# TimZaman/dotaclient

Hardware: NVIDIA H100
Metric: optimizer_steps_per_sec (higher is better)
Workload: dtype f32

## Files before the change

### dotaclient_b200/csrc/gemm_tf32x3.cu

```cuda
#include "dc_common.cuh"
#include "unit_basic.cuh"

namespace {

constexpr int BM = 128, BN = 128, BK = 32;
constexpr int kStages = 2;
constexpr int kTileBytes = BM * BK * 4;
constexpr int kStageBytes = 4 * kTileBytes;
constexpr int kProducerThreads = 128;
constexpr int kProducerGroups = kStages;
constexpr int kConsumerWarp0 = 4 * kProducerGroups;
constexpr int kConsumerThreads = 256;
constexpr int kThreads = kConsumerWarp0 * 32 + kConsumerThreads;
constexpr int kLdS = BN + 8;
constexpr int kDIn = kUnitFeatures;
constexpr size_t kOffStaging = (size_t)kStages * kStageBytes;
constexpr size_t kOffBars = kOffStaging + (size_t)BM * kLdS * 4;
constexpr size_t kSmemBytes = kOffBars + 128 + 1024 ;

#define DC_ACC8(b) "+f"(d[b]), "+f"(d[b + 1]), "+f"(d[b + 2]), "+f"(d[b + 3]), "+f"(d[b + 4]), "+f"(d[b + 5]), "+f"(d[b + 6]), "+f"(d[b + 7])
__device__ __forceinline__ void wgmma_m64n128k8(float (&d)[64], uint64_t desc_a, uint64_t desc_b) {
    asm volatile(
        "{\n\t.reg .pred p;\n\tsetp.ne.b32 p, %66, 0;\n\t"
        "wgmma.mma_async.sync.aligned.m64n128k8.f32.tf32.tf32 "
        "{%0, %1, %2, %3, %4, %5, %6, %7, %8, %9, %10, %11, %12, %13, %14, %15, "
        "%16, %17, %18, %19, %20, %21, %22, %23, %24, %25, %26, %27, %28, %29, %30, %31, "
        "%32, %33, %34, %35, %36, %37, %38, %39, %40, %41, %42, %43, %44, %45, %46, %47, "
        "%48, %49, %50, %51, %52, %53, %54, %55, %56, %57, %58, %59, %60, %61, %62, %63}, "
        "%64, %65, p, 1, 1;\n\t}\n"
        : DC_ACC8(0), DC_ACC8(8), DC_ACC8(16), DC_ACC8(24), DC_ACC8(32), DC_ACC8(40), DC_ACC8(48), DC_ACC8(56)
        : "l"(desc_a), "l"(desc_b), "r"(1));
}
#undef DC_ACC8

__device__ __forceinline__ void mma_stage(float (&d)[64], uint32_t stage_base, int wg) {
    const uint64_t a_hi = dc_wgmma_desc(stage_base + wg * (64 * 128)), a_lo = dc_wgmma_desc(stage_base + kTileBytes + wg * (64 * 128));
    const uint64_t b_hi = dc_wgmma_desc(stage_base + 2 * kTileBytes), b_lo = dc_wgmma_desc(stage_base + 3 * kTileBytes);
#pragma unroll
    for (int i = 0; i < 64; ++i) dc_reg_fence(d[i]);
    dc_wgmma_fence();
#pragma unroll
    for (int ks = 0; ks < BK / 8; ++ks) {
        const uint64_t adv = (uint64_t)(ks * 2);
        wgmma_m64n128k8(d, a_lo + adv, b_hi + adv);
        wgmma_m64n128k8(d, a_hi + adv, b_lo + adv);
        wgmma_m64n128k8(d, a_hi + adv, b_hi + adv);
    }
    dc_wgmma_commit();
    dc_wgmma_wait0();
#pragma unroll
    for (int i = 0; i < 64; ++i) dc_reg_fence(d[i]);
}

__device__ __forceinline__ void consume(float (&d)[64], unsigned char *tiles, uint64_t *full, uint64_t *empty, uint32_t &c, int n,
                                       int wg, int lane) {
#pragma unroll
    for (int i = 0; i < 64; ++i) d[i] = 0.f;
    for (int kc = 0; kc < n; ++kc, ++c) {
        const int s = c % kStages;
        dc_mbar_wait(&full[s], (c / kStages) & 1);
        __syncwarp();
        mma_stage(d, dc_smem_u32(tiles + (size_t)s * kStageBytes), wg);
        __syncwarp();
        if (lane == 0) dc_mbar_arrive(&empty[s]);
    }
}

__device__ __forceinline__ void consumer_sync() { asm volatile("bar.sync 1, %0;" ::"n"(kConsumerThreads) : "memory"); }

__device__ __forceinline__ void stage_acc(const float (&d)[64], float *S, int ct) {
    const int wg = ct >> 7, w = (ct >> 5) & 3, lane = ct & 31;
    const int r0 = 64 * wg + 16 * w + (lane >> 2), c0 = 2 * (lane & 3);
#pragma unroll
    for (int i = 0; i < 64; i += 2) {
        const int row = r0 + 8 * ((i >> 1) & 1), col = 8 * (i >> 2) + c0;
        *reinterpret_cast<float2 *>(S + row * kLdS + col) = make_float2(d[i], d[i + 1]);
    }
}

__device__ __forceinline__ void init_ring(uint64_t *bars) {
    if (threadIdx.x == 0) {
        for (int s = 0; s < kStages; ++s) { dc_mbar_init(&bars[s], 4); dc_mbar_init(&bars[kStages + s], kConsumerThreads / 32); }
        asm volatile("fence.mbarrier_init.release.cluster;" ::: "memory");
    }
    __syncthreads();
}
__device__ __forceinline__ unsigned char *smem_base(unsigned char *raw) {
    return reinterpret_cast<unsigned char *>((reinterpret_cast<uintptr_t>(raw) + 1023) & ~(uintptr_t)1023);
}
template <typename F>
__device__ __forceinline__ void produce(uint64_t *full, uint64_t *empty, uint32_t c, int lane, F &&store) {
    const int s = c % kStages;
    dc_mbar_wait(&empty[s], ((c / kStages) & 1) ^ 1);
    store(s);
    asm volatile("fence.proxy.async.shared::cta;" ::: "memory");
    __syncwarp();
    if (lane == 0) dc_mbar_arrive(&full[s]);
}

__device__ __forceinline__ void tile_load_k(const float *__restrict__ src, int ld, int row0, int rows_total, int k0, int t,
                                            float4 (&v)[8]) {
    const int c = t & 7, r0 = t >> 3;
#pragma unroll
    for (int i = 0; i < 8; ++i) {
        const int r = r0 + 16 * i;
        v[i] = (row0 + r < rows_total) ? __ldg(reinterpret_cast<const float4 *>(src + (size_t)(row0 + r) * ld + k0) + c)
                                       : make_float4(0.f, 0.f, 0.f, 0.f);
    }
}
__device__ __forceinline__ void tile_store_k(const float4 (&v)[8], unsigned char *dst_hi, unsigned char *dst_lo, int t) {
    const int c = t & 7, r0 = t >> 3;
#pragma unroll
    for (int i = 0; i < 8; ++i) {
        const int r = r0 + 16 * i;
        const int off = r * 128 + ((c ^ (r & 7)) << 4);
        float4 hi, lo;
        hi.x = dc_tf32_rna(v[i].x); hi.y = dc_tf32_rna(v[i].y); hi.z = dc_tf32_rna(v[i].z); hi.w = dc_tf32_rna(v[i].w);
        lo.x = v[i].x - hi.x; lo.y = v[i].y - hi.y; lo.z = v[i].z - hi.z; lo.w = v[i].w - hi.w;
        *reinterpret_cast<float4 *>(dst_hi + off) = hi;
        *reinterpret_cast<float4 *>(dst_lo + off) = lo;
    }
}

template <int NU>
struct DembRaw {
    static constexpr int kP = NU == 16 ? 1 : 2;
    static constexpr int kU = NU == 16 ? 8 : NU;
    float4 d[kP], d2[kP], a[kP];
    uint32_t am[kP];
    float g[kP][kU];
    bool ok[kP];
};
template <>
struct DembRaw<1> {
    float4 v[8];
};

template <int NU>
__device__ __forceinline__ void demb_fetch(DembRaw<NU> &raw, const float *__restrict__ dx, const float *__restrict__ dx2, int ld_dx,
                                           const uint8_t *__restrict__ argmax, const float *__restrict__ dl, int ld_dl,
                                           const float *__restrict__ att, int tok0, int n_tok, int k0, int t) {
    const float4 zero4 = make_float4(0.f, 0.f, 0.f, 0.f);
    if constexpr (NU == 1) {
        const int c = t & 7, r0 = t >> 3;
#pragma unroll
        for (int i = 0; i < 8; ++i) {
            const int n = tok0 + r0 + 16 * i;
            const bool ok = n < n_tok;
            const size_t nn = (size_t)min(n, n_tok - 1);
            float4 d = dx != nullptr ? __ldg(reinterpret_cast<const float4 *>(dx + nn * ld_dx + k0) + c) : zero4;
            if (dx2 != nullptr) {
                const float4 d2 = __ldg(reinterpret_cast<const float4 *>(dx2 + nn * ld_dx + k0) + c);
                d.x += d2.x; d.y += d2.y; d.z += d2.z; d.w += d2.w;
            }
            const float4 a4 = dl != nullptr ? __ldg(reinterpret_cast<const float4 *>(att + nn * 128 + k0) + c) : zero4;
            const float gl = dl != nullptr ? __ldg(dl + nn * ld_dl) : 0.f;
            raw.v[i] = ok ? make_float4(fmaf(gl, a4.x, d.x), fmaf(gl, a4.y, d.y), fmaf(gl, a4.z, d.z), fmaf(gl, a4.w, d.w)) : zero4;
        }
    } else {
        constexpr int kTileToks = (BM - BM % NU) / NU;
#pragma unroll
        for (int k = 0; k < DembRaw<NU>::kP; ++k) {
            const int p = t + kProducerThreads * k;
            const int c = p & 7, tokl = NU == 16 ? p >> 4 : p >> 3;
            const int u0 = NU == 16 ? ((p >> 3) & 1) * 8 : 0;
            const bool active = tokl < kTileToks;
            const int n = tok0 + tokl;
            raw.ok[k] = active && n < n_tok;
            const size_t nn = (size_t)min(n, n_tok - 1);
            float4 d = (active && dx != nullptr) ? __ldg(reinterpret_cast<const float4 *>(dx + nn * ld_dx + k0) + c) : zero4;
            const float4 d2 = (active && dx2 != nullptr) ? __ldg(reinterpret_cast<const float4 *>(dx2 + nn * ld_dx + k0) + c) : zero4;
            if constexpr (NU == 16) {
                raw.d2[k] = d2;
            } else {
                d.x += d2.x; d.y += d2.y; d.z += d2.z; d.w += d2.w;
            }
            raw.d[k] = d;
            raw.am[k] = (active && dx != nullptr) ? __ldg(reinterpret_cast<const uint32_t *>(argmax + nn * 128 + k0) + c) : 0u;
            raw.a[k] = (active && dl != nullptr) ? __ldg(reinterpret_cast<const float4 *>(att + nn * 128 + k0) + c) : zero4;
#pragma unroll
            for (int j = 0; j < DembRaw<NU>::kU; ++j) raw.g[k][j] = (active && dl != nullptr) ? __ldg(dl + nn * ld_dl + u0 + j) : 0.f;
        }
    }
}

__device__ __forceinline__ void store_hi_lo(unsigned char *dst_hi, unsigned char *dst_lo, int off, float4 o) {
    float4 hi, lo;
    hi.x = dc_tf32_rna(o.x); hi.y = dc_tf32_rna(o.y); hi.z = dc_tf32_rna(o.z); hi.w = dc_tf32_rna(o.w);
    lo.x = o.x - hi.x; lo.y = o.y - hi.y; lo.z = o.z - hi.z; lo.w = o.w - hi.w;
    *reinterpret_cast<float4 *>(dst_hi + off) = hi;
    *reinterpret_cast<float4 *>(dst_lo + off) = lo;
}

template <int NU>
__device__ __forceinline__ void demb_store(const DembRaw<NU> &raw, unsigned char *dst_hi, unsigned char *dst_lo, int t) {
    if constexpr (NU == 1) {
        tile_store_k(raw.v, dst_hi, dst_lo, t);
    } else {
        constexpr int kTileRows = BM - BM % NU, kTileToks = kTileRows / NU;
        const float4 zero4 = make_float4(0.f, 0.f, 0.f, 0.f);
#pragma unroll
        for (int k = 0; k < DembRaw<NU>::kP; ++k) {
            const int p = t + kProducerThreads * k;
            const int c = p & 7, tokl = NU == 16 ? p >> 4 : p >> 3;
            const int u0 = NU == 16 ? ((p >> 3) & 1) * 8 : 0;
            if (tokl < kTileToks) {
                float4 d = raw.d[k];
                if constexpr (NU == 16) { d.x += raw.d2[k].x; d.y += raw.d2[k].y; d.z += raw.d2[k].z; d.w += raw.d2[k].w; }
                const float4 a = raw.a[k];
                const uint32_t am = raw.am[k];
#pragma unroll
                for (int j = 0; j < DembRaw<NU>::kU; ++j) {
                    const int u = u0 + j, r = tokl * NU + u;
                    const float gl = raw.g[k][j];
                    float4 o;
                    o.x = fmaf(gl, a.x, (int)(am & 0xffu) == u ? d.x : 0.f);
                    o.y = fmaf(gl, a.y, (int)((am >> 8) & 0xffu) == u ? d.y : 0.f);
                    o.z = fmaf(gl, a.z, (int)((am >> 16) & 0xffu) == u ? d.z : 0.f);
                    o.w = fmaf(gl, a.w, (int)(am >> 24) == u ? d.w : 0.f);
                    store_hi_lo(dst_hi, dst_lo, r * 128 + ((c ^ (r & 7)) << 4), raw.ok[k] ? o : zero4);
                }
            }
        }
        if constexpr (kTileRows < BM) {
            if (t < (BM - kTileRows) * 8) {
                const int r = kTileRows + (t >> 3), c = t & 7;
                store_hi_lo(dst_hi, dst_lo, r * 128 + ((c ^ (r & 7)) << 4), zero4);
            }
        }
    }
}

__device__ __forceinline__ void store_row_k(const float (&v)[32], unsigned char *dst_hi, unsigned char *dst_lo, int row) {
#pragma unroll
    for (int c = 0; c < 8; ++c) {
        const int off = row * 128 + ((c ^ (row & 7)) << 4);
        float4 hi, lo;
        hi.x = dc_tf32_rna(v[4 * c]); hi.y = dc_tf32_rna(v[4 * c + 1]); hi.z = dc_tf32_rna(v[4 * c + 2]); hi.w = dc_tf32_rna(v[4 * c + 3]);
        lo.x = v[4 * c] - hi.x; lo.y = v[4 * c + 1] - hi.y; lo.z = v[4 * c + 2] - hi.z; lo.w = v[4 * c + 3] - hi.w;
        *reinterpret_cast<float4 *>(dst_hi + off) = hi;
        *reinterpret_cast<float4 *>(dst_lo + off) = lo;
    }
}

__global__ void __launch_bounds__(kThreads, 1) gemm_tf32x3_kernel(const float *__restrict__ A, int lda,
                                                                  const float *__restrict__ B, int ldb,
                                                                  const float *__restrict__ bias, float *__restrict__ C,
                                                                  int ldc, int M, int N, int K, int relu, int ksplit,
                                                                  long long c_split_stride) {
    constexpr int kTileRows = BM;
    extern __shared__ unsigned char smem_raw[];
    unsigned char *tiles = smem_base(smem_raw);
    float *S = reinterpret_cast<float *>(tiles + kOffStaging);
    uint64_t *full = reinterpret_cast<uint64_t *>(tiles + kOffBars), *empty = full + kStages;

    const int warp = threadIdx.x >> 5, lane = threadIdx.x & 31;
    const int m_blocks = (M + kTileRows - 1) / kTileRows, n_blocks = (N + BN - 1) / BN, k_chunks = K / BK / ksplit;
    const int tiles_mn = m_blocks * n_blocks, tiles_total = tiles_mn * ksplit;
    init_ring(full);

    if (warp < kConsumerWarp0) {
        const int t = threadIdx.x & (kProducerThreads - 1), g = warp >> 2;
        uint32_t c = 0;
        for (int tile = blockIdx.x; tile < tiles_total; tile += gridDim.x) {
            const int tmn = tile % tiles_mn, kc0 = (tile / tiles_mn) * k_chunks;
            const int m0 = (tmn / n_blocks) * kTileRows, n0 = (tmn % n_blocks) * BN;
            for (int kc = 0; kc < k_chunks; ++kc, ++c) {
                if ((int)(c % kProducerGroups) != g) continue;
                float4 va[8], vb[8];
                tile_load_k(A, lda, m0, M, (kc0 + kc) * BK, t, va);
                tile_load_k(B, ldb, n0, N, (kc0 + kc) * BK, t, vb);
                produce(full, empty, c, lane, [&](int s) {
                    unsigned char *st = tiles + (size_t)s * kStageBytes;
                    tile_store_k(va, st, st + kTileBytes, t);
                    tile_store_k(vb, st + 2 * kTileBytes, st + 3 * kTileBytes, t);
                });
            }
        }
    } else {
        const int ct = threadIdx.x - kConsumerWarp0 * 32, wg = ct >> 7, cw = ct >> 5;
        float d[64];
        uint32_t c = 0;
        for (int tile = blockIdx.x; tile < tiles_total; tile += gridDim.x) {
            const int tmn = tile % tiles_mn, sp = tile / tiles_mn;
            const int m0 = (tmn / n_blocks) * kTileRows, n0 = (tmn % n_blocks) * BN;
            consume(d, tiles, full, empty, c, k_chunks, wg, lane);
            consumer_sync();
            stage_acc(d, S, ct);
            consumer_sync();
            const bool lane_in = n0 + 4 * lane < N;
            const bool has_bias = bias != nullptr && sp == 0 && lane_in;
            const float4 b4 = has_bias ? __ldg(reinterpret_cast<const float4 *>(bias + n0) + lane) : make_float4(0.f, 0.f, 0.f, 0.f);
            float *cbase = C + (size_t)sp * (size_t)c_split_stride + n0 + 4 * lane;
            for (int r = cw; lane_in && r < BM && m0 + r < M; r += kConsumerThreads / 32) {
                float4 v = *reinterpret_cast<const float4 *>(S + r * kLdS + 4 * lane);
                if (has_bias) { v.x += b4.x; v.y += b4.y; v.z += b4.z; v.w += b4.w; }
                if (relu) { v.x = fmaxf(v.x, 0.f); v.y = fmaxf(v.y, 0.f); v.z = fmaxf(v.z, 0.f); v.w = fmaxf(v.w, 0.f); }
                *reinterpret_cast<float4 *>(cbase + (size_t)(m0 + r) * ldc) = v;
            }
        }
    }
}

constexpr int kWsRows = 64;
constexpr int kWsStages = 8;
constexpr int kWsChunkBytes = kWsRows * BK * 4;
constexpr int kWsThreads = kConsumerThreads + 128;
constexpr int kWsLdS = 40;
constexpr size_t kWsOffRing = (size_t)4 * 2 * kTileBytes;
constexpr size_t kWsOffStaging = kWsOffRing + (size_t)kWsStages * kWsChunkBytes;
constexpr size_t kWsOffBars = kWsOffStaging + (size_t)(kConsumerThreads / 32) * 16 * kWsLdS * 4;
constexpr size_t kWsSmemBytes = kWsOffBars + 2 * kWsStages * 8 + 1024 ;
constexpr size_t kWsOffUnits = kWsOffBars + 2 * kWsStages * 8;
constexpr size_t kWsGenSmemBytes = kWsOffUnits + (size_t)4 * kWsRows * kDIn * 4 + 1024 ;
static_assert(kWsSmemBytes <= 227 * 1024 && kWsGenSmemBytes <= 227 * 1024, "weight-stationary GEMM exceeds the shared-memory opt-in");
static_assert(kWsOffUnits % 16 == 0, "unit rows are staged with 16-byte stores");

struct GenA {
    const float *units, *w_b, *b_b;
    float *basic_out;
    uint32_t *mask_out;
};

__device__ __forceinline__ void cp_async16(uint32_t dst, const void *src, uint32_t src_bytes) {
    asm volatile("cp.async.cg.shared.global [%0], [%1], 16, %2;" ::"r"(dst), "l"(src), "r"(src_bytes) : "memory");
}
__device__ __forceinline__ void cp_async_arrive(uint64_t *bar) {
    asm volatile("cp.async.mbarrier.arrive.noinc.shared::cta.b64 [%0];" ::"r"(dc_smem_u32(bar)) : "memory");
}

#define DC_ACC8(b) "+f"(d[b]), "+f"(d[b + 1]), "+f"(d[b + 2]), "+f"(d[b + 3]), "+f"(d[b + 4]), "+f"(d[b + 5]), "+f"(d[b + 6]), "+f"(d[b + 7])
__device__ __forceinline__ void wgmma_m64n128k8_rs(float (&d)[64], uint32_t a0, uint32_t a1, uint32_t a2, uint32_t a3, uint64_t desc_b) {
    asm volatile(
        "{\n\t.reg .pred p;\n\tsetp.ne.b32 p, %69, 0;\n\t"
        "wgmma.mma_async.sync.aligned.m64n128k8.f32.tf32.tf32 "
        "{%0, %1, %2, %3, %4, %5, %6, %7, %8, %9, %10, %11, %12, %13, %14, %15, "
        "%16, %17, %18, %19, %20, %21, %22, %23, %24, %25, %26, %27, %28, %29, %30, %31, "
        "%32, %33, %34, %35, %36, %37, %38, %39, %40, %41, %42, %43, %44, %45, %46, %47, "
        "%48, %49, %50, %51, %52, %53, %54, %55, %56, %57, %58, %59, %60, %61, %62, %63}, "
        "{%64, %65, %66, %67}, %68, p, 1, 1;\n\t}\n"
        : DC_ACC8(0), DC_ACC8(8), DC_ACC8(16), DC_ACC8(24), DC_ACC8(32), DC_ACC8(40), DC_ACC8(48), DC_ACC8(56)
        : "r"(a0), "r"(a1), "r"(a2), "r"(a3), "l"(desc_b), "r"(1));
}
#undef DC_ACC8

__device__ __forceinline__ void ws_fetch(float (&v)[16], const float *chunk, int rlo, int rhi, bool hi_ok, int q) {
#pragma unroll
    for (int ks = 0; ks < BK / 8; ++ks) {
#pragma unroll
        for (int h = 0; h < 2; ++h) {
            const int j = 2 * ks + h;
            v[4 * ks + 2 * h] = chunk[rlo * BK + ((j ^ (rlo & 7)) << 2) + q];
            v[4 * ks + 2 * h + 1] = hi_ok ? chunk[rhi * BK + ((j ^ (rhi & 7)) << 2) + q] : 0.f;
        }
    }
}

template <int NU, bool kGenA>
__global__ void __launch_bounds__(kWsThreads, 1) gemm_ws_kernel(const float *__restrict__ A, int lda,
                                                                const float *__restrict__ B, int ldb,
                                                                const float *__restrict__ bias, float *__restrict__ C,
                                                                int ldc, int M, int N, int K, int relu,
                                                                float *__restrict__ C_copy, uint8_t *__restrict__ argmax, GenA gen) {
    constexpr int kWarpRows = NU == 5 ? 15 : 16;
    constexpr int kTileRows = 4 * kWarpRows;
    extern __shared__ unsigned char smem_raw[];
    unsigned char *sm = smem_base(smem_raw);
    unsigned char *ring = sm + kWsOffRing;
    uint64_t *full = reinterpret_cast<uint64_t *>(sm + kWsOffBars), *empty = full + kWsStages;

    const int warp = threadIdx.x >> 5, lane = threadIdx.x & 31;
    const int n_blocks = (N + BN - 1) / BN, m_blocks = (M + kTileRows - 1) / kTileRows, k_chunks = K / BK;
    const int n0 = (blockIdx.x % n_blocks) * BN, mb0 = blockIdx.x / n_blocks, mstride = gridDim.x / n_blocks;
    if (threadIdx.x == 0) {
        for (int s = 0; s < kWsStages; ++s) { dc_mbar_init(&full[s], kGenA ? 1 : 128); dc_mbar_init(&empty[s], 4); }
        asm volatile("fence.mbarrier_init.release.cluster;" ::: "memory");
    }
    __syncthreads();

    if constexpr (kGenA) if (warp >= kConsumerThreads / 32) {
        const int kc = warp - kConsumerThreads / 32, ch = lane & 7, r0 = lane >> 3;
        const int j0 = kc * BK + 4 * ch;
        float wb[4][kDIn], bb[4];
// ... 338 lines not shown
            tile_load_k(Wt, BN, 0, BN, kc * BK, t, vb);
            tile_store_k(vb, sm + (size_t)kc * 2 * kTileBytes, sm + (size_t)kc * 2 * kTileBytes + kTileBytes, t);
        }
        asm volatile("fence.proxy.async.shared::cta;" ::: "memory");
        consumer_sync();
        const uint32_t w_base = dc_smem_u32(sm) + wg * (64 * 128), ring_base = dc_smem_u32(ring), u_base = dc_smem_u32(sm_u);
        const int j_lo = 64 * wg + 16 * w4 + (lane >> 2);
        const uint32_t bit_lo = 1u << (j_lo >> 2), bit_hi = bit_lo << 2;
        const uint32_t *mrow = sm_mask + (j_lo & 3) * kDgMaskLd + 2 * q4;
        float acc[8];
#pragma unroll
        for (int i = 0; i < 8; ++i) acc[i] = 0.f;
        float d[64];
        uint32_t c = 0;
        int it = 0;
        for (int mb = blockIdx.x; mb < m_blocks; mb += gridDim.x, ++it) {
#pragma unroll
            for (int i = 0; i < 64; ++i) d[i] = 0.f;
#pragma unroll 1
            for (int kc = 0; kc < k_chunks; ++kc, ++c) {
                const int s = c % kStages;
                dc_mbar_wait(&full[s], (c / kStages) & 1);
#pragma unroll
                for (int i = 0; i < 64; ++i) dc_reg_fence(d[i]);
                dc_wgmma_fence();
                const uint64_t a_hi = dc_wgmma_desc(w_base + kc * 2 * kTileBytes), a_lo = dc_wgmma_desc(w_base + kc * 2 * kTileBytes + kTileBytes);
                const uint64_t b_hi = dc_wgmma_desc(ring_base + s * kDgStageBytes), b_lo = dc_wgmma_desc(ring_base + s * kDgStageBytes + kTileBytes);
#pragma unroll
                for (int ks = 0; ks < BK / 8; ++ks) {
                    const uint64_t adv = (uint64_t)(ks * 2);
                    wgmma_m64n128k8(d, a_hi + adv, b_lo + adv);
                    wgmma_m64n128k8(d, a_lo + adv, b_hi + adv);
                    wgmma_m64n128k8(d, a_hi + adv, b_hi + adv);
                }
                dc_wgmma_commit();
                if (kc > 0) {
                    wgmma_wait1();
                    __syncwarp();
                    if (lane == 0) dc_mbar_arrive(&empty[(c - 1) % kStages]);
                }
            }
            dc_wgmma_wait0();
#pragma unroll
            for (int i = 0; i < 64; ++i) dc_reg_fence(d[i]);
            __syncwarp();
            if (lane == 0) dc_mbar_arrive(&empty[(c - 1) % kStages]);

            dc_mbar_wait(ufull, it & 1);
            uint32_t ghi[2][4], glo[2][4];
#pragma unroll
            for (int q = 0; q < BM / 8; ++q) {
                const int b = q & 1;
                const uint2 mw = *reinterpret_cast<const uint2 *>(mrow + 8 * q);
                const float gv[4] = {(mw.x & bit_lo) ? d[4 * q] : 0.f, (mw.x & bit_hi) ? d[4 * q + 2] : 0.f,
                                     (mw.y & bit_lo) ? d[4 * q + 1] : 0.f, (mw.y & bit_hi) ? d[4 * q + 3] : 0.f};
#pragma unroll
                for (int e = 0; e < 4; ++e) {
                    const float h = dc_tf32_rna(gv[e]);
                    ghi[b][e] = __float_as_uint(h);
                    glo[b][e] = __float_as_uint(gv[e] - h);
                }
                dc_wgmma_fence();
                const uint64_t u_hi = dc_wgmma_desc(u_base + (q >> 2) * kDgUTile) + 2 * (q & 3);
                const uint64_t u_lo = dc_wgmma_desc(u_base + (BM / BK + (q >> 2)) * kDgUTile) + 2 * (q & 3);
                wgmma_m64n16k8_rs(acc, glo[b], u_hi);
                wgmma_m64n16k8_rs(acc, ghi[b], u_lo);
                wgmma_m64n16k8_rs(acc, ghi[b], u_hi);
                dc_wgmma_commit();
                wgmma_wait1();
#pragma unroll
                for (int e = 0; e < 4; ++e) asm volatile("" : "+r"(ghi[b ^ 1][e]), "+r"(glo[b ^ 1][e])::"memory");
            }
            dc_wgmma_wait0();
#pragma unroll
            for (int i = 0; i < 8; ++i) dc_reg_fence(acc[i]);
            __syncwarp();
            if (lane == 0) dc_mbar_arrive(uempty);
        }
        float *pp = partial + (size_t)blockIdx.x * BN * (kDIn + 1);
#pragma unroll
        for (int i = 0; i < 8; ++i) {
            const int j = j_lo + 8 * ((i >> 1) & 1), n = 8 * (i >> 2) + 2 * q4 + (i & 1);
            if (n <= kDIn) pp[j * (kDIn + 1) + n] = acc[i];
        }
    }
}

constexpr int kWgStages = 4;
constexpr int kWgLdX = BN + 8;
constexpr int kWgStageBytes = 2 * kTileBytes + BK * kWgLdX * 4;
constexpr size_t kWgOffColsum = (size_t)kWgStages * kWgStageBytes;
constexpr size_t kWgOffBars = kWgOffColsum + 2 * BM * 4;
constexpr size_t kWgSmemBytes = kWgOffBars + 2 * kWgStages * 8 + 1024 ;
static_assert(kWgStageBytes % 1024 == 0, "the swizzled dY^T tiles need 1024-byte aligned slots");
static_assert(kWgSmemBytes <= 227 * 1024, "weight-gradient GEMM exceeds the shared-memory opt-in");

__device__ __forceinline__ float lds_f32(uint32_t addr) {
    float v;
    asm volatile("ld.shared.f32 %0, [%1];" : "=f"(v) : "r"(addr) : "memory");
    return v;
}

template <int NU>
__global__ void __launch_bounds__(kThreads, 1) gemm_wgrad_kernel(const float *__restrict__ dY, int ldy,
                                                                 const float *__restrict__ dY2,
                                                                 const uint8_t *__restrict__ argmax,
                                                                 const float *__restrict__ X, int ldx, int T, int No,
                                                                 int Ni, int nsplit, float *__restrict__ part_w,
                                                                 float *__restrict__ part_b) {
    constexpr int kTPC = NU > 0 ? BK / NU : 0;
    constexpr int kRPC = NU > 0 ? kTPC * NU : BK;
    extern __shared__ unsigned char smem_raw[];
    unsigned char *ring = smem_base(smem_raw);
    float *colsum_s = reinterpret_cast<float *>(ring + kWgOffColsum);
    uint64_t *full = reinterpret_cast<uint64_t *>(ring + kWgOffBars), *empty = full + kWgStages;

    const int warp = threadIdx.x >> 5, lane = threadIdx.x & 31;
    const int n_blocks = (Ni + BN - 1) / BN, tiles_mn = ((No + BM - 1) / BM) * n_blocks;
    const int tile = blockIdx.x % tiles_mn, split = blockIdx.x / tiles_mn;
    const int m0 = (tile / n_blocks) * BM, n0 = (tile % n_blocks) * BN;
    const int chunks_total = (T + kRPC - 1) / kRPC;
    const int my_chunks = split < chunks_total ? (chunks_total - split + nsplit - 1) / nsplit : 0;
    if (threadIdx.x == 0) {
        for (int s = 0; s < kWgStages; ++s) { dc_mbar_init(&full[s], kProducerThreads + 4); dc_mbar_init(&empty[s], kConsumerThreads / 32); }
        asm volatile("fence.mbarrier_init.release.cluster;" ::: "memory");
    }
    __syncthreads();

    if (warp < kConsumerWarp0) {
        const int g = warp >> 2, t = threadIdx.x & (kProducerThreads - 1), o = m0 + t;
        const bool o_in = o < No;
        const int xc = t & 31;
        const bool xc_in = n0 + 4 * xc < Ni;
        float cs = 0.f;
        for (int j = g; j < my_chunks; j += kProducerGroups) {
            float va[32];
            if constexpr (NU > 0) {
                const int tok0 = (split + j * nsplit) * kTPC, n_tok = T / NU;
                float dv[kTPC];
                int am[kTPC];
#pragma unroll
                for (int k = 0; k < kTPC; ++k) {
                    const bool ok = tok0 + k < n_tok;
                    const size_t at = (size_t)(tok0 + k) * ldy + o;
                    dv[k] = ok ? __ldg(dY + at) : 0.f;
                    if (ok && dY2 != nullptr) dv[k] += __ldg(dY2 + at);
                    am[k] = ok ? (int)__ldg(argmax + (size_t)(tok0 + k) * 128 + o) : 255;
                }
#pragma unroll
                for (int i = 0; i < 32; ++i) va[i] = (i < kRPC && am[i / NU] == i % NU) ? dv[i / NU] : 0.f;
            } else {
                const int t0 = (split + j * nsplit) * BK;
                const float *p = dY + (size_t)t0 * ldy + o;
#pragma unroll
                for (int i = 0; i < 32; ++i) va[i] = (o_in && t0 + i < T) ? __ldg(p + (size_t)i * ldy) : 0.f;
            }
#pragma unroll
            for (int i = 0; i < 32; ++i) cs += va[i];
            const int t0 = (split + j * nsplit) * kRPC, tend = min(T, t0 + kRPC);
            const int s = j % kWgStages;
            dc_mbar_wait(&empty[s], ((j / kWgStages) & 1) ^ 1);
            unsigned char *st = ring + (size_t)s * kWgStageBytes;
            const uint32_t xs = dc_smem_u32(st + 2 * kTileBytes);
#pragma unroll
            for (int r = 0; r < BK / 4; ++r) {
                const int row = (t >> 5) + 4 * r;
// ... 60 lines not shown
#pragma unroll
        for (int i = 0; i < 64; ++i) dc_reg_fence(d[i]);
        float *pt = part_w + ((size_t)split * tiles_mn + tile) * BM * BN + rlo;
#pragma unroll
        for (int k = 0; k < 64; ++k) pt[(size_t)(8 * (k >> 2) + 2 * q + (k & 1)) * BN + 8 * ((k >> 1) & 1)] = d[k];
    }
    __syncthreads();
    if (part_b != nullptr && n0 == 0 && threadIdx.x < 128 && m0 + (int)threadIdx.x < No)
        part_b[(size_t)split * No + m0 + threadIdx.x] = colsum_s[threadIdx.x] + colsum_s[128 + threadIdx.x];
}

constexpr int kRedRows = 8;
__global__ void __launch_bounds__(32 * kRedRows) wgrad_reduce_kernel(const float *__restrict__ part_w, const float *__restrict__ part_b,
                                                                     int nsplit, int No, int Ni, float *__restrict__ dW, int ldw,
                                                                     float *__restrict__ db, int accumulate) {
    __shared__ float4 sh[kRedRows][32];
    const int x = threadIdx.x & 31, y = threadIdx.x >> 5;
    const int n_blocks = (Ni + BN - 1) / BN, tiles_mn = ((No + BM - 1) / BM) * n_blocks;
    const int total4 = No * Ni / 4, bias4 = db != nullptr ? No / 4 : 0;
    const int idx = blockIdx.x * 32 + x;
    const float *src = nullptr;
    float *dst = nullptr;
    size_t stride = 0;
    if (idx < total4) {
        const int o = (idx * 4) / Ni, i = (idx * 4) % Ni;
        const int tile = (o / BM) * n_blocks + i / BN;
        src = part_w + ((size_t)tile * BM + o % BM) * BN + i % BN;
        stride = (size_t)tiles_mn * BM * BN;
        dst = dW + (size_t)o * ldw + i;
    } else if (idx < total4 + bias4) {
        src = part_b + (size_t)(idx - total4) * 4;
        stride = (size_t)No;
        dst = db + (size_t)(idx - total4) * 4;
    }
    float4 acc = make_float4(0.f, 0.f, 0.f, 0.f);
    if (src != nullptr) {
#pragma unroll 4
        for (int s = y; s < nsplit; s += kRedRows) {
            const float4 v = __ldg(reinterpret_cast<const float4 *>(src + (size_t)s * stride));
            acc.x += v.x; acc.y += v.y; acc.z += v.z; acc.w += v.w;
        }
    }
    sh[y][x] = acc;
    __syncthreads();
    if (y == 0 && dst != nullptr) {
        float4 t = accumulate ? *reinterpret_cast<const float4 *>(dst) : make_float4(0.f, 0.f, 0.f, 0.f);
#pragma unroll
        for (int r = 0; r < kRedRows; ++r) { t.x += sh[r][x].x; t.y += sh[r][x].y; t.z += sh[r][x].z; t.w += sh[r][x].w; }
        *reinterpret_cast<float4 *>(dst) = t;
    }
}

}

extern "C" int dc_gemm_tf32x3_supported(int64_t M, int N, int K) { return M > 0 && N > 0 && K > 0 && N % 32 == 0 && K % BK == 0; }

template <int NU, bool kGenA = false>
static int launch_ws(const float *A, int lda, const float *B, int ldb, const float *bias, float *C, int ldc, int M, int N,
                     int K, int relu, float *C_copy, uint8_t *argmax, cudaStream_t st, GenA gen = GenA{}) {
    const int tile_rows = NU == 5 ? 60 : kWsRows;
    const int n_blocks = (N + BN - 1) / BN, m_blocks = (M + tile_rows - 1) / tile_rows;
    int per_block = dc_sm_count() / n_blocks;
    if (per_block < 1) per_block = 1;
    if (per_block > m_blocks) per_block = m_blocks;
    const size_t smem = kGenA ? kWsGenSmemBytes : kWsSmemBytes;
    DC_CUDA(cudaFuncSetAttribute(gemm_ws_kernel<NU, kGenA>, cudaFuncAttributeMaxDynamicSharedMemorySize, (int)smem));
    gemm_ws_kernel<NU, kGenA><<<n_blocks * per_block, kWsThreads, smem, st>>>(A, lda, B, ldb, bias, C, ldc, M, N, K, relu, C_copy,
                                                                             argmax, gen);
    DC_LAUNCH_OK();
    return DC_OK;
}

extern "C" int dc_gemm_tf32x3(const float *A, int lda, const float *B, int ldb, const float *bias, float *C, int ldc,
                              int64_t M, int N, int K, int relu, dc_stream_t stream) {
    DC_REQUIRE(A && B && C, DC_EINVAL, "dc_gemm_tf32x3: null pointer");
    DC_REQUIRE(dc_gemm_tf32x3_supported(M, N, K) && M < (1ll << 31) - BM, DC_EUNSUPPORTED,
               "dc_gemm_tf32x3: need N %% 32 == 0 and K %% 32 == 0 (M=%lld N=%d K=%d)", (long long)M, N, K);
    DC_REQUIRE(lda >= K && ldb >= K && ldc >= N && lda % 4 == 0 && ldb % 4 == 0 && ldc % 4 == 0, DC_EINVAL,
               "dc_gemm_tf32x3: leading dimensions must be >= extent and multiples of 4 floats");
    DC_REQUIRE(((uintptr_t)A & 15) == 0 && ((uintptr_t)B & 15) == 0 && ((uintptr_t)C & 15) == 0 && (!bias || ((uintptr_t)bias & 15) == 0),
               DC_EINVAL, "dc_gemm_tf32x3: pointers must be 16-byte aligned");
    if (K <= 4 * BK) return launch_ws<0>(A, lda, B, ldb, bias, C, ldc, (int)M, N, K, relu, nullptr, nullptr, dc_cu_stream(stream));
    const int tiles = (int)((M + BM - 1) / BM) * ((N + BN - 1) / BN);
    DC_CUDA(cudaFuncSetAttribute(gemm_tf32x3_kernel, cudaFuncAttributeMaxDynamicSharedMemorySize, (int)kSmemBytes));
    const int grid = tiles < dc_sm_count() ? tiles : dc_sm_count();
    gemm_tf32x3_kernel<<<grid, kThreads, kSmemBytes, dc_cu_stream(stream)>>>(A, lda, B, ldb, bias, C, ldc, (int)M, N, K, relu, 1, 0);
    DC_LAUNCH_OK();
    return DC_OK;
}

int dc_gemm_tf32x3_splitk(const float *A, int lda, const float *B, int ldb, float *part, int64_t M, int N, int K, int ksplit,
                          bool first_call, cudaStream_t st) {
    DC_REQUIRE(A && B && part && ksplit >= 1 && N % BN == 0 && K % (BK * ksplit) == 0 && M > 0, DC_EINVAL,
               "dc_gemm_tf32x3_splitk: bad arguments (M=%lld N=%d K=%d ksplit=%d)", (long long)M, N, K, ksplit);
    if (first_call)
        DC_CUDA(cudaFuncSetAttribute(gemm_tf32x3_kernel, cudaFuncAttributeMaxDynamicSharedMemorySize, (int)kSmemBytes));
    const int tiles = (int)((M + BM - 1) / BM) * (N / BN) * ksplit;
    const int grid = tiles < dc_sm_count() ? tiles : dc_sm_count();
    gemm_tf32x3_kernel<<<grid, kThreads, kSmemBytes, st>>>(A, lda, B, ldb, nullptr, part, N, (int)M, N, K, 0, ksplit, (long long)M * N);
    DC_LAUNCH_OK();
    return DC_OK;
}

static int wgrad_tiles(int No, int Ni) { return ((No + BM - 1) / BM) * ((Ni + BN - 1) / BN); }

static int wgrad_splits(int No, int Ni) {
    const int tiles_mn = wgrad_tiles(No, Ni);
    const int n = dc_sm_count() / tiles_mn;
    return n < 1 ? 1 : n;
}

extern "C" size_t dc_gemm_wgrad_workspace_bytes(int No, int Ni) {
    if (No <= 0 || Ni <= 0 || No % 32 || Ni % 32) return 0;
    const int nsplit = wgrad_splits(No, Ni);
    return ((size_t)nsplit * wgrad_tiles(No, Ni) * BM * BN + (size_t)nsplit * No) * sizeof(float);
}

extern "C" int dc_gemm_wgrad_tf32x3(const float *dY, int ldy, const float *X, int ldx, int64_t T, int No, int Ni, float *dW,
                                    int ldw, float *db, int accumulate, void *workspace, dc_stream_t stream) {
    DC_REQUIRE(dY && X && dW && workspace, DC_EINVAL, "dc_gemm_wgrad_tf32x3: null pointer");
    DC_REQUIRE(T > 0 && T < (1ll << 31) - BK && No > 0 && Ni > 0 && No % 32 == 0 && Ni % 32 == 0, DC_EUNSUPPORTED,
               "dc_gemm_wgrad_tf32x3: need No %% 32 == 0 and Ni %% 32 == 0 (T=%lld No=%d Ni=%d)", (long long)T, No, Ni);
    DC_REQUIRE(ldy >= No && ldx >= Ni && ldw >= Ni && ldy % 4 == 0 && ldx % 4 == 0 && ldw % 4 == 0, DC_EINVAL,
               "dc_gemm_wgrad_tf32x3: bad leading dimension");
    DC_REQUIRE(((uintptr_t)dY & 15) == 0 && ((uintptr_t)X & 15) == 0 && ((uintptr_t)dW & 15) == 0 && ((uintptr_t)workspace & 15) == 0 &&
                   ((uintptr_t)db & 15) == 0,
               DC_EINVAL, "dc_gemm_wgrad_tf32x3: pointers must be 16-byte aligned");
    const int tiles_mn = wgrad_tiles(No, Ni), nsplit = wgrad_splits(No, Ni);
    float *part_w = reinterpret_cast<float *>(workspace);
    float *part_b = db ? part_w + (size_t)nsplit * tiles_mn * BM * BN : nullptr;
    cudaStream_t st = dc_cu_stream(stream);
    DC_CUDA(cudaFuncSetAttribute(gemm_wgrad_kernel<0>, cudaFuncAttributeMaxDynamicSharedMemorySize, (int)kWgSmemBytes));
    gemm_wgrad_kernel<0><<<tiles_mn * nsplit, kThreads, kWgSmemBytes, st>>>(dY, ldy, nullptr, nullptr, X, ldx, (int)T, No, Ni,
                                                                                      nsplit, part_w, part_b);
    DC_LAUNCH_OK();
    const int total4 = No * Ni / 4 + (db ? No / 4 : 0);
    wgrad_reduce_kernel<<<(total4 + 31) / 32, 32 * kRedRows, 0, st>>>(part_w, part_b, nsplit, No, Ni, dW, ldw, db, accumulate);
    DC_LAUNCH_OK();
    return DC_OK;
}

extern "C" int dc_gemm_unit_max(const float *basic, const float *w, const float *bias, float *xmax, float *xmax_copy, int ld_x,
                                uint8_t *argmax, int64_t n_tokens, int n_units, dc_stream_t stream) {
    DC_REQUIRE(basic && w && bias && xmax && argmax && n_tokens > 0, DC_EINVAL, "dc_gemm_unit_max: null pointer / empty input");
    DC_REQUIRE(n_units == 5 || n_units == 16, DC_EUNSUPPORTED, "dc_gemm_unit_max: n_units=%d (5 or 16; 1-unit groups are plain GEMMs)", n_units);
    DC_REQUIRE(ld_x >= BN && n_tokens * n_units < (1ll << 31) - BM, DC_EINVAL, "dc_gemm_unit_max: bad ld_x / size");
    DC_REQUIRE(((uintptr_t)basic & 15) == 0 && ((uintptr_t)w & 15) == 0, DC_EINVAL, "dc_gemm_unit_max: pointers must be 16-byte aligned");
    const int M = (int)(n_tokens * n_units);
    cudaStream_t st = dc_cu_stream(stream);
    if (n_units == 5) return launch_ws<5>(basic, BN, w, BN, bias, xmax, ld_x, M, BN, BN, 0, xmax_copy, argmax, st);
    return launch_ws<16>(basic, BN, w, BN, bias, xmax, ld_x, M, BN, BN, 0, xmax_copy, argmax, st);
}

extern "C" int dc_unit_embed_fwd_mask(const float *units, const float *w_b, const float *b_b, float *basic_out, uint32_t *mask_out,
                                      const float *w, const float *bias, float *xmax, float *xmax_copy, int ld_x, uint8_t *argmax,
                                      int64_t n_tokens, int n_units, dc_stream_t stream) {
    DC_REQUIRE(units && w_b && b_b && w && bias && xmax && n_tokens > 0, DC_EINVAL, "dc_unit_embed_fwd: null pointer / empty input");
    DC_REQUIRE(n_units == 1 || n_units == 5 || n_units == 16, DC_EUNSUPPORTED, "dc_unit_embed_fwd: n_units=%d (1, 5 or 16)", n_units);
    DC_REQUIRE(n_units == 1 ? (argmax == nullptr && xmax_copy == nullptr) : argmax != nullptr, DC_EINVAL,
               "dc_unit_embed_fwd: the arg-max (and the copy) go with the max-pool of n_units 5 and 16 only");
    DC_REQUIRE(ld_x >= BN && ld_x % 4 == 0 && n_tokens * n_units < (1ll << 31) - BM, DC_EINVAL, "dc_unit_embed_fwd: bad ld_x / size");
    DC_REQUIRE(((uintptr_t)units & 15) == 0 && ((uintptr_t)basic_out & 15) == 0 && ((uintptr_t)w & 15) == 0 && ((uintptr_t)bias & 15) == 0 &&
                   ((uintptr_t)xmax & 15) == 0 && ((uintptr_t)xmax_copy & 15) == 0 && ((uintptr_t)mask_out & 15) == 0,
               DC_EINVAL, "dc_unit_embed_fwd: units, basic_out, mask_out, w, bias, xmax, xmax_copy must be 16-byte aligned");
    const int M = (int)(n_tokens * n_units);
    const GenA gen{units, w_b, b_b, basic_out, mask_out};
    cudaStream_t st = dc_cu_stream(stream);
    if (n_units == 1) return launch_ws<0, true>(nullptr, BN, w, BN, bias, xmax, ld_x, M, BN, BN, 0, nullptr, nullptr, st, gen);
    if (n_units == 5) return launch_ws<5, true>(nullptr, BN, w, BN, bias, xmax, ld_x, M, BN, BN, 0, xmax_copy, argmax, st, gen);
    return launch_ws<16, true>(nullptr, BN, w, BN, bias, xmax, ld_x, M, BN, BN, 0, xmax_copy, argmax, st, gen);
}

extern "C" int dc_unit_embed_fwd(const float *units, const float *w_b, const float *b_b, float *basic_out, const float *w, const float *bias,
                                 float *xmax, float *xmax_copy, int ld_x, uint8_t *argmax, int64_t n_tokens, int n_units,
                                 dc_stream_t stream) {
    return dc_unit_embed_fwd_mask(units, w_b, b_b, basic_out, nullptr, w, bias, xmax, xmax_copy, ld_x, argmax, n_tokens, n_units, stream);
}

extern "C" int dc_unit_dgrad_fused_mask(const float *d_xmax, const float *d_xmax2, int ld_dx, const uint8_t *argmax, const float *dlogits,
                                        int ld_dl, const float *att, const float *w_t, const float *units, const uint32_t *mask,
                                        const float *w_b, const float *b_b, int64_t n_tokens, int n_units, float *dw_b, float *db_b,
                                        int accumulate, void *workspace, dc_stream_t stream) {
// ... 72 lines not shown
```

Measured before the change: 78.96.

## Replace TF32x3 GEMM with register-A streaming kernel using cp.async and deeper ring

```diff
diff --git a/dotaclient_b200/csrc/gemm_tf32x3.cu b/dotaclient_b200/csrc/gemm_tf32x3.cu
--- a/dotaclient_b200/csrc/gemm_tf32x3.cu
+++ b/dotaclient_b200/csrc/gemm_tf32x3.cu
@@ -6,17 +6,12 @@
 constexpr int BM = 128, BN = 128, BK = 32;
 constexpr int kStages = 2;
 constexpr int kTileBytes = BM * BK * 4;
-constexpr int kStageBytes = 4 * kTileBytes;
 constexpr int kProducerThreads = 128;
-constexpr int kProducerGroups = kStages;
+constexpr int kProducerGroups = 2;
 constexpr int kConsumerWarp0 = 4 * kProducerGroups;
 constexpr int kConsumerThreads = 256;
 constexpr int kThreads = kConsumerWarp0 * 32 + kConsumerThreads;
-constexpr int kLdS = BN + 8;
 constexpr int kDIn = kUnitFeatures;
-constexpr size_t kOffStaging = (size_t)kStages * kStageBytes;
-constexpr size_t kOffBars = kOffStaging + (size_t)BM * kLdS * 4;
-constexpr size_t kSmemBytes = kOffBars + 128 + 1024 ;
 
 #define DC_ACC8(b) "+f"(d[b]), "+f"(d[b + 1]), "+f"(d[b + 2]), "+f"(d[b + 3]), "+f"(d[b + 4]), "+f"(d[b + 5]), "+f"(d[b + 6]), "+f"(d[b + 7])
 __device__ __forceinline__ void wgmma_m64n128k8(float (&d)[64], uint64_t desc_a, uint64_t desc_b) {
@@ -33,50 +28,7 @@
 }
 #undef DC_ACC8
 
-__device__ __forceinline__ void mma_stage(float (&d)[64], uint32_t stage_base, int wg) {
-    const uint64_t a_hi = dc_wgmma_desc(stage_base + wg * (64 * 128)), a_lo = dc_wgmma_desc(stage_base + kTileBytes + wg * (64 * 128));
-    const uint64_t b_hi = dc_wgmma_desc(stage_base + 2 * kTileBytes), b_lo = dc_wgmma_desc(stage_base + 3 * kTileBytes);
-#pragma unroll
-    for (int i = 0; i < 64; ++i) dc_reg_fence(d[i]);
-    dc_wgmma_fence();
-#pragma unroll
-    for (int ks = 0; ks < BK / 8; ++ks) {
-        const uint64_t adv = (uint64_t)(ks * 2);
-        wgmma_m64n128k8(d, a_lo + adv, b_hi + adv);
-        wgmma_m64n128k8(d, a_hi + adv, b_lo + adv);
-        wgmma_m64n128k8(d, a_hi + adv, b_hi + adv);
-    }
-    dc_wgmma_commit();
-    dc_wgmma_wait0();
-#pragma unroll
-    for (int i = 0; i < 64; ++i) dc_reg_fence(d[i]);
-}
-
-__device__ __forceinline__ void consume(float (&d)[64], unsigned char *tiles, uint64_t *full, uint64_t *empty, uint32_t &c, int n,
-                                       int wg, int lane) {
-#pragma unroll
-    for (int i = 0; i < 64; ++i) d[i] = 0.f;
-    for (int kc = 0; kc < n; ++kc, ++c) {
-        const int s = c % kStages;
-        dc_mbar_wait(&full[s], (c / kStages) & 1);
-        __syncwarp();
-        mma_stage(d, dc_smem_u32(tiles + (size_t)s * kStageBytes), wg);
-        __syncwarp();
-        if (lane == 0) dc_mbar_arrive(&empty[s]);
-    }
-}
-
 __device__ __forceinline__ void consumer_sync() { asm volatile("bar.sync 1, %0;" ::"n"(kConsumerThreads) : "memory"); }
-
-__device__ __forceinline__ void stage_acc(const float (&d)[64], float *S, int ct) {
-    const int wg = ct >> 7, w = (ct >> 5) & 3, lane = ct & 31;
-    const int r0 = 64 * wg + 16 * w + (lane >> 2), c0 = 2 * (lane & 3);
-#pragma unroll
-    for (int i = 0; i < 64; i += 2) {
-        const int row = r0 + 8 * ((i >> 1) & 1), col = 8 * (i >> 2) + c0;
-        *reinterpret_cast<float2 *>(S + row * kLdS + col) = make_float2(d[i], d[i + 1]);
-    }
-}
 
 __device__ __forceinline__ void init_ring(uint64_t *bars) {
     if (threadIdx.x == 0) {
@@ -240,65 +192,6 @@
         lo.x = v[4 * c] - hi.x; lo.y = v[4 * c + 1] - hi.y; lo.z = v[4 * c + 2] - hi.z; lo.w = v[4 * c + 3] - hi.w;
         *reinterpret_cast<float4 *>(dst_hi + off) = hi;
         *reinterpret_cast<float4 *>(dst_lo + off) = lo;
-    }
-}
-
-__global__ void __launch_bounds__(kThreads, 1) gemm_tf32x3_kernel(const float *__restrict__ A, int lda,
-                                                                  const float *__restrict__ B, int ldb,
-                                                                  const float *__restrict__ bias, float *__restrict__ C,
-                                                                  int ldc, int M, int N, int K, int relu, int ksplit,
-                                                                  long long c_split_stride) {
-    constexpr int kTileRows = BM;
-    extern __shared__ unsigned char smem_raw[];
-    unsigned char *tiles = smem_base(smem_raw);
-    float *S = reinterpret_cast<float *>(tiles + kOffStaging);
-    uint64_t *full = reinterpret_cast<uint64_t *>(tiles + kOffBars), *empty = full + kStages;
-
-    const int warp = threadIdx.x >> 5, lane = threadIdx.x & 31;
-    const int m_blocks = (M + kTileRows - 1) / kTileRows, n_blocks = (N + BN - 1) / BN, k_chunks = K / BK / ksplit;
-    const int tiles_mn = m_blocks * n_blocks, tiles_total = tiles_mn * ksplit;
-    init_ring(full);
-
-    if (warp < kConsumerWarp0) {
-        const int t = threadIdx.x & (kProducerThreads - 1), g = warp >> 2;
-        uint32_t c = 0;
-        for (int tile = blockIdx.x; tile < tiles_total; tile += gridDim.x) {
-            const int tmn = tile % tiles_mn, kc0 = (tile / tiles_mn) * k_chunks;
-            const int m0 = (tmn / n_blocks) * kTileRows, n0 = (tmn % n_blocks) * BN;
-            for (int kc = 0; kc < k_chunks; ++kc, ++c) {
-                if ((int)(c % kProducerGroups) != g) continue;
-                float4 va[8], vb[8];
-                tile_load_k(A, lda, m0, M, (kc0 + kc) * BK, t, va);
-                tile_load_k(B, ldb, n0, N, (kc0 + kc) * BK, t, vb);
-                produce(full, empty, c, lane, [&](int s) {
-                    unsigned char *st = tiles + (size_t)s * kStageBytes;
-                    tile_store_k(va, st, st + kTileBytes, t);
-                    tile_store_k(vb, st + 2 * kTileBytes, st + 3 * kTileBytes, t);
-                });
-            }
-        }
-    } else {
-        const int ct = threadIdx.x - kConsumerWarp0 * 32, wg = ct >> 7, cw = ct >> 5;
-        float d[64];
-        uint32_t c = 0;
-        for (int tile = blockIdx.x; tile < tiles_total; tile += gridDim.x) {
-            const int tmn = tile % tiles_mn, sp = tile / tiles_mn;
-            const int m0 = (tmn / n_blocks) * kTileRows, n0 = (tmn % n_blocks) * BN;
-            consume(d, tiles, full, empty, c, k_chunks, wg, lane);
-            consumer_sync();
-            stage_acc(d, S, ct);
-            consumer_sync();
-            const bool lane_in = n0 + 4 * lane < N;
-            const bool has_bias = bias != nullptr && sp == 0 && lane_in;
-            const float4 b4 = has_bias ? __ldg(reinterpret_cast<const float4 *>(bias + n0) + lane) : make_float4(0.f, 0.f, 0.f, 0.f);
-            float *cbase = C + (size_t)sp * (size_t)c_split_stride + n0 + 4 * lane;
-            for (int r = cw; lane_in && r < BM && m0 + r < M; r += kConsumerThreads / 32) {
-                float4 v = *reinterpret_cast<const float4 *>(S + r * kLdS + 4 * lane);
-                if (has_bias) { v.x += b4.x; v.y += b4.y; v.z += b4.z; v.w += b4.w; }
-                if (relu) { v.x = fmaxf(v.x, 0.f); v.y = fmaxf(v.y, 0.f); v.z = fmaxf(v.z, 0.f); v.w = fmaxf(v.w, 0.f); }
-                *reinterpret_cast<float4 *>(cbase + (size_t)(m0 + r) * ldc) = v;
-            }
-        }
     }
 }
 
@@ -803,6 +696,136 @@
         for (int i = 0; i < 8; ++i) {
             const int j = j_lo + 8 * ((i >> 1) & 1), n = 8 * (i >> 2) + 2 * q4 + (i & 1);
             if (n <= kDIn) pp[j * (kDIn + 1) + n] = acc[i];
+        }
+    }
+}
+
+constexpr int kRsStages = 4;
+constexpr int kRsStageBytes = 3 * kTileBytes;
+constexpr size_t kRsOffBars = (size_t)kRsStages * kRsStageBytes;
+constexpr size_t kRsSmemBytes = kRsOffBars + 2 * kRsStages * 8 + 1024 ;
+static_assert(kRsSmemBytes <= 227 * 1024, "streaming-weight GEMM exceeds the shared-memory opt-in");
+
+__global__ void __launch_bounds__(kThreads, 1) gemm_stream_kernel(const float *__restrict__ A, int lda,
+                                                                  const float *__restrict__ B, int ldb,
+                                                                  const float *__restrict__ bias, float *__restrict__ C,
+                                                                  int ldc, int M, int N, int K, int relu, int ksplit,
+                                                                  long long c_split_stride) {
+    extern __shared__ unsigned char smem_raw[];
+    unsigned char *ring = smem_base(smem_raw);
+    uint64_t *full = reinterpret_cast<uint64_t *>(ring + kRsOffBars), *empty = full + kRsStages;
+
+    const int warp = threadIdx.x >> 5, lane = threadIdx.x & 31;
+    const int m_blocks = (M + BM - 1) / BM, n_blocks = (N + BN - 1) / BN, k_chunks = K / BK / ksplit;
+    const int tiles_mn = m_blocks * n_blocks, tiles_total = tiles_mn * ksplit;
+    if (threadIdx.x == 0) {
+        for (int s = 0; s < kRsStages; ++s) { dc_mbar_init(&full[s], kProducerThreads + 4); dc_mbar_init(&empty[s], kConsumerThreads / 32); }
+        asm volatile("fence.mbarrier_init.release.cluster;" ::: "memory");
+    }
+    __syncthreads();
+
+    if (warp < kConsumerWarp0) {
+        const int t = threadIdx.x & (kProducerThreads - 1), g = warp >> 2, ch = t & 7, r0 = t >> 3;
+        const uint32_t a_off = r0 * 128 + ((ch ^ (r0 & 7)) << 4);
+        uint32_t c = 0;
+        for (int tile = blockIdx.x; tile < tiles_total; tile += gridDim.x) {
+            const int tmn = tile % tiles_mn, kc0 = (tile / tiles_mn) * k_chunks;
+            const int m0 = (tmn / n_blocks) * BM, n0 = (tmn % n_blocks) * BN;
+            for (int kc = 0; kc < k_chunks; ++kc, ++c) {
+                if ((int)(c % kProducerGroups) != g) continue;
+                const int k0 = (kc0 + kc) * BK;
+                float4 vb[8];
+                tile_load_k(B, ldb, n0, N, k0, t, vb);
+                const int s = c % kRsStages;
+                dc_mbar_wait(&empty[s], ((c / kRsStages) & 1) ^ 1);
+                unsigned char *st = ring + (size_t)s * kRsStageBytes;
+                const uint32_t a_dst = dc_smem_u32(st + 2 * kTileBytes) + a_off;
+#pragma unroll
+                for (int i = 0; i < BM / 16; ++i) {
+                    const int r = r0 + 16 * i;
+                    const bool ok = m0 + r < M;
+                    cp_async16(a_dst + 16 * i * 128, A + (ok ? (size_t)(m0 + r) * lda : 0) + k0 + 4 * ch, ok ? 16u : 0u);
+                }
+                cp_async_arrive(&full[s]);
+                tile_store_k(vb, st, st + kTileBytes, t);
+                asm volatile("fence.proxy.async.shared::cta;" ::: "memory");
+                __syncwarp();
+                if (lane == 0) dc_mbar_arrive(&full[s]);
+            }
+        }
+        asm volatile("cp.async.wait_all;" ::: "memory");
+        return;
+    }
+
+    const int wg = (warp - kConsumerWarp0) >> 2, w4 = warp & 3, q = lane & 3, g8 = lane >> 2;
+    const int rlo = 16 * w4 + g8, rhi = rlo + 8;
+    float d[64];
+    uint32_t ahi[2][4] = {}, alo[2][4] = {};
+    uint32_t c = 0;
+    for (int tile = blockIdx.x; tile < tiles_total; tile += gridDim.x) {
+        const int tmn = tile % tiles_mn, sp = tile / tiles_mn;
+        const int m0 = (tmn / n_blocks) * BM, n0 = (tmn % n_blocks) * BN;
+#pragma unroll
+        for (int i = 0; i < 64; ++i) d[i] = 0.f;
+        for (int kc = 0; kc < k_chunks; ++kc, ++c) {
+            const int s = c % kRsStages;
+            dc_mbar_wait(&full[s], (c / kRsStages) & 1);
+            unsigned char *st = ring + (size_t)s * kRsStageBytes;
+            const float *chunk = reinterpret_cast<const float *>(st + 2 * kTileBytes) + 64 * wg * BK;
+            const uint64_t b_hi = dc_wgmma_desc(dc_smem_u32(st)), b_lo = dc_wgmma_desc(dc_smem_u32(st + kTileBytes));
+#pragma unroll
+            for (int ks = 0; ks < BK / 8; ++ks) {
+                const int b = ks & 1;
+                float v[4];
+#pragma unroll
+                for (int h = 0; h < 2; ++h) {
+                    const int j = 2 * ks + h;
+                    v[2 * h] = chunk[rlo * BK + ((j ^ (rlo & 7)) << 2) + q];
+                    v[2 * h + 1] = chunk[rhi * BK + ((j ^ (rhi & 7)) << 2) + q];
+                }
+#pragma unroll
+                for (int e = 0; e < 4; ++e) {
+                    const float h = dc_tf32_rna(v[e]);
+                    ahi[b][e] = __float_as_uint(h);
+                    alo[b][e] = __float_as_uint(v[e] - h);
+                }
+                dc_wgmma_fence();
+                const uint64_t adv = (uint64_t)(ks * 2);
+                wgmma_m64n128k8_rs(d, alo[b][0], alo[b][1], alo[b][2], alo[b][3], b_hi + adv);
+                wgmma_m64n128k8_rs(d, ahi[b][0], ahi[b][1], ahi[b][2], ahi[b][3], b_lo + adv);
+                wgmma_m64n128k8_rs(d, ahi[b][0], ahi[b][1], ahi[b][2], ahi[b][3], b_hi + adv);
+                dc_wgmma_commit();
+                wgmma_wait1();
+#pragma unroll
+                for (int e = 0; e < 4; ++e) asm volatile("" : "+r"(ahi[b ^ 1][e]), "+r"(alo[b ^ 1][e])::"memory");
+                if (ks == 0 && kc > 0) {
+                    __syncwarp();
+                    if (lane == 0) dc_mbar_arrive(&empty[(c - 1) % kRsStages]);
+                }
+            }
+        }
+        dc_wgmma_wait0();
+#pragma unroll
+        for (int i = 0; i < 64; ++i) dc_reg_fence(d[i]);
+        __syncwarp();
+        if (lane == 0) dc_mbar_arrive(&empty[(c - 1) % kRsStages]);
+
+        const int row_lo = m0 + 64 * wg + rlo, row_hi = row_lo + 8;
+        float *cs = C + (size_t)sp * (size_t)c_split_stride;
+        float *c_lo = cs + (size_t)row_lo * ldc, *c_hi = cs + (size_t)row_hi * ldc;
+        const bool has_bias = bias != nullptr && sp == 0;
+#pragma unroll
+        for (int g = 0; g < BN / 8; ++g) {
+            const int col = n0 + 8 * g + 2 * q;
+            const bool in = col < N;
+            float2 lo = make_float2(d[4 * g], d[4 * g + 1]), hi = make_float2(d[4 * g + 2], d[4 * g + 3]);
+            if (has_bias && in) {
+                const float2 b2 = __ldg(reinterpret_cast<const float2 *>(bias + col));
+                lo.x += b2.x; lo.y += b2.y; hi.x += b2.x; hi.y += b2.y;
+            }
+            if (relu) { lo.x = fmaxf(lo.x, 0.f); lo.y = fmaxf(lo.y, 0.f); hi.x = fmaxf(hi.x, 0.f); hi.y = fmaxf(hi.y, 0.f); }
+            if (in && row_lo < M) *reinterpret_cast<float2 *>(c_lo + col) = lo;
+            if (in && row_hi < M) *reinterpret_cast<float2 *>(c_hi + col) = hi;
         }
     }
 }
@@ -1029,9 +1052,9 @@
                DC_EINVAL, "dc_gemm_tf32x3: pointers must be 16-byte aligned");
     if (K <= 4 * BK) return launch_ws<0>(A, lda, B, ldb, bias, C, ldc, (int)M, N, K, relu, nullptr, nullptr, dc_cu_stream(stream));
     const int tiles = (int)((M + BM - 1) / BM) * ((N + BN - 1) / BN);
-    DC_CUDA(cudaFuncSetAttribute(gemm_tf32x3_kernel, cudaFuncAttributeMaxDynamicSharedMemorySize, (int)kSmemBytes));
+    DC_CUDA(cudaFuncSetAttribute(gemm_stream_kernel, cudaFuncAttributeMaxDynamicSharedMemorySize, (int)kRsSmemBytes));
     const int grid = tiles < dc_sm_count() ? tiles : dc_sm_count();
-    gemm_tf32x3_kernel<<<grid, kThreads, kSmemBytes, dc_cu_stream(stream)>>>(A, lda, B, ldb, bias, C, ldc, (int)M, N, K, relu, 1, 0);
+    gemm_stream_kernel<<<grid, kThreads, kRsSmemBytes, dc_cu_stream(stream)>>>(A, lda, B, ldb, bias, C, ldc, (int)M, N, K, relu, 1, 0);
     DC_LAUNCH_OK();
     return DC_OK;
 }
@@ -1041,10 +1064,10 @@
     DC_REQUIRE(A && B && part && ksplit >= 1 && N % BN == 0 && K % (BK * ksplit) == 0 && M > 0, DC_EINVAL,
                "dc_gemm_tf32x3_splitk: bad arguments (M=%lld N=%d K=%d ksplit=%d)", (long long)M, N, K, ksplit);
     if (first_call)
-        DC_CUDA(cudaFuncSetAttribute(gemm_tf32x3_kernel, cudaFuncAttributeMaxDynamicSharedMemorySize, (int)kSmemBytes));
+        DC_CUDA(cudaFuncSetAttribute(gemm_stream_kernel, cudaFuncAttributeMaxDynamicSharedMemorySize, (int)kRsSmemBytes));
     const int tiles = (int)((M + BM - 1) / BM) * (N / BN) * ksplit;
     const int grid = tiles < dc_sm_count() ? tiles : dc_sm_count();
-    gemm_tf32x3_kernel<<<grid, kThreads, kSmemBytes, st>>>(A, lda, B, ldb, nullptr, part, N, (int)M, N, K, 0, ksplit, (long long)M * N);
+    gemm_stream_kernel<<<grid, kThreads, kRsSmemBytes, st>>>(A, lda, B, ldb, nullptr, part, N, (int)M, N, K, 0, ksplit, (long long)M * N);
     DC_LAUNCH_OK();
     return DC_OK;
 }
```

Result: no change. 79.22 (median of 6 runs) (+0.3%).
